# Mozobo/Ocean-Simulation

Measured on AMD Instinct MI355X. Metric: ocean-surface frames/sec (4x1024^2 cascades), higher is better.
Workload: dtype f32; 1 GPU; cfg3: 4 x 1024^2 cascades, displacement + derivatives + Jacobian foam; n=1024, cascades=4, tiles_per_gpu=1, tiles_total=1, schedule=fused (pass A + pass B), parallelism=independent oceans over 1 GPU(s), no collective

## Files before the change

### ocean-simulation_amd/csrc/fftq.hip

```cpp
#include "fft_engine.h"
#include "spectrum_math.h"

namespace ocean {
namespace {

__device__ __forceinline__ float2 hsum(float2 a, float2 b) { return make_float2((a.x + b.x) * 0.5f, (a.y - b.y) * 0.5f); }
__device__ __forceinline__ float2 hdif(float2 a, float2 b) { return make_float2((a.x - b.x) * 0.5f, (a.y + b.y) * 0.5f); }

struct QTex {
    float2 q[3];
};

__device__ __forceinline__ void q_planes(const Planes4& o, const Planes4& om, QTex& a, QTex& b) {
    const float2 h2 = hsum(o.p[1], om.p[1]), h3 = hsum(o.p[2], om.p[2]);
    const float2 a3 = hdif(o.p[2], om.p[2]), h4 = hsum(o.p[3], om.p[3]);
    a.q[0] = o.p[0];
    b.q[0] = om.p[0];
    a.q[1] = make_float2(h2.x - h3.y, h2.y + h3.x);
    b.q[1] = make_float2(h2.x + h3.y, h3.x - h2.y);
    a.q[2] = make_float2(a3.y - h4.y, h4.x - a3.x);
    b.q[2] = make_float2(a3.y + h4.y, a3.x + h4.x);
}

__device__ __forceinline__ void q_fast(float2 h, float4 w, QTex& a, QTex& b) {
    const float c1x = -w.z * w.y, c1y = w.x * w.y;
    a.q[0] = make_float2(c1x * h.x - c1y * h.y, c1x * h.y + c1y * h.x);
    b.q[0] = make_float2(-(c1x * h.x + c1y * h.y), c1x * h.y - c1y * h.x);
    const float s2a = 1.0f - w.x, s2b = 1.0f + w.x;
    a.q[1] = make_float2(s2a * h.x, s2a * h.y);
    b.q[1] = make_float2(s2b * h.x, -s2b * h.y);
    const float kk = w.x * w.x * w.y;
    const float t1 = w.z - kk, t2 = -w.z - kk;
    a.q[2] = make_float2(-t1 * h.y, t1 * h.x);
    b.q[2] = make_float2(t2 * h.y, t2 * h.x);
}

__device__ __forceinline__ float2 q4_minus(const Planes4& o, const Planes4& om, float kz) {
    const float2 a2 = hdif(o.p[1], om.p[1]), a4 = hdif(o.p[3], om.p[3]);
    return make_float2(a2.y + a4.x + kz * o.p[0].y, -a2.x + a4.y - kz * o.p[0].x);
}
__device__ __forceinline__ float2 q4_full(const Planes4& o, const Planes4& om) {
    const float2 a2 = hdif(o.p[1], om.p[1]), a4 = hdif(o.p[3], om.p[3]);
    return make_float2(a2.y + a4.x, -a2.x + a4.y);
}

template <int N>
__device__ __forceinline__ float4 mirror_factors(int x, int y, const WaveBand& wb, float g, float time) {
    const float kx = (float)(x - N / 2) * wb.dk, kz = (float)(y - N / 2) * wb.dk;
    const float kmag = sqrtf(kx * kx + kz * kz);
    if (!(kmag >= wb.lo && kmag <= wb.hi)) return make_float4(1.0f, 0.0f, 1.0f, 0.0f);
    const Phase e = evolve_phase(sqrtf(g * kmag), time);
    return make_float4(e.ex, e.ey, __builtin_amdgcn_rcpf(kmag), 0.0f);
}

__device__ __forceinline__ float2* q_side(const DevView& v, int u) { return v.qside + (size_t)u * 2 * v.n; }

template <int N, bool BAND = false, int WT = 0, bool OFF32 = true>
__global__ __launch_bounds__(N / 4) __attribute__((amdgpu_waves_per_eu(N == 1024 ? 3 : 1, N == 1024 ? 3 : 10))) void
k_pass_aq(DevView v, float time, int items) {
    constexpr int R0 = 4, NJ = N / R0;
    constexpr int IPU = N / 2 + 1;
    using TW = StageTw<N, R0>;
    using E = Engine<N, 4, false, true, R0, TW, kElems>;
    constexpr int T = E::THREADS;
    static_assert(T == NJ && E::R0 == R0, "lane j <-> stage-0 butterfly j");
    constexpr int W = WT ? WT : inter_w(N);
    constexpr int TILES = N / W;
    constexpr int NSL = N / E::RL;
    static_assert(NSL % W == 0, "tile-major emit");
    __shared__ float2 lds[E::LDS_ELEMS];
    __shared__ float2 twl[TW::kLdsEntries];
    TW::load(twl, v.tw, threadIdx.x, T);
    const float2* tws = TW::table(twl, v.tw);
    __shared__ WaveBand band[kMaxCascades];
    if ((int)threadIdx.x < v.C) band[threadIdx.x] = wave_band(v.casc + threadIdx.x * 5);
    const int j = (int)threadIdx.x;
    const int jm = (NJ - j) & (NJ - 1);
    const bool j0 = (j == 0);
    auto rows_of = [&](int it, int& u, int& y1, int& y2) {
        u = it / IPU;
        y1 = it - u * IPU;
        y2 = (N - y1) & (N - 1);
    };
    auto load_pair = [&](int it, float2 (&a)[R0], float2 (&b)[R0]) {
        int u, y1, y2;
        rows_of(it, u, y1, y2);
        const float2* r1 = v.h0k + ((size_t)u * N + y1) * N;
        const float2* r2 = v.h0k + ((size_t)u * N + y2) * N;
#pragma unroll
        for (int r = 0; r < R0; ++r) {
            a[r] = r1[j + r * NJ];
            b[r] = r2[(N - j - r * NJ) & (N - 1)];
        }
    };
    auto unmirror = [&](const float2* mir, float2* out) {
#pragma unroll
        for (int r2 = 0; r2 < R0; ++r2) out[r2] = j0 ? mir[(R0 - r2) & (R0 - 1)] : mir[R0 - 1 - r2];
    };
    auto put = [&](int b, int jb, const float2* x) {
        float2* dst = lds + E::lidx(b, jb * R0);
#pragma unroll
        for (int q = 0; q < R0; ++q) dst[E::loff(q, 1)] = x[q];
    };
    float2 A[R0], B[R0], An[R0], Bn[R0];
    int it = blockIdx.x;
    if (it < items) load_pair(it, A, B);
    __syncthreads();
    for (; it < items; it += gridDim.x) {
        const int next = it + gridDim.x;
        if (next < items) load_pair(next, An, Bn);
        int u, y1, y2;
        rows_of(it, u, y1, y2);
        const WaveBand wb = band[(u + v.c0) % v.C];
        const bool self = (y1 == y2);
        const Win wunit = make_win(v.tplane + (size_t)u * TILES * N * W, 0);
        float2 g[6][R0];
        {
            float2 mir[3][R0];
#pragma unroll
            for (int r = 0; r < R0; ++r) {
                const float4 f = mirror_factors<N>(j + r * NJ, y1, wb, v.gravity, time);
                const float4 wd = make_float4((float)(j + r * NJ - N / 2) * wb.dk, f.z, (float)(y1 - N / 2) * wb.dk, 0.0f);
                const float2 h = evolve_h(make_float4(A[r].x, A[r].y, B[r].x, -B[r].y), Phase{f.x, f.y});
                QTex qa, qb;
                if (y1 != 0 && !(r == 0 && j0)) {
                    q_fast(h, wd, qa, qb);
                } else {
                    const float4 wm = make_float4((j0 && r == 0) ? wd.x : -wd.x, wd.y, y1 ? -wd.z : wd.z, wd.w);
                    const Planes4 o = planes_of(h, wd), om = planes_of(make_float2(h.x, -h.y), wm);
                    q_planes(o, om, qa, qb);
                    if (y1 == 0) qb.q[2] = q4_full(o, om);
                    if (r == 0 && j0) {
                        float2* side = q_side(v, u);
                        side[y1] = q4_minus(o, om, wd.z);
                        side[y2] = q4_minus(om, o, wm.z);
// ... 297 lines not shown
            const int mm = jj + q * NSL;
            if (b == 6) {
                if (y1 == 0) q_side(v, u)[N + mm] = val;
                return;
            }
            if (b >= 3 && self) return;
            const int p = b >= 3 ? b - 3 : b;
            const int y = b >= 3 ? y2 : y1;
            if constexpr (OFF32) {
                const unsigned e = (unsigned)p * (unsigned)v.inter_stride + ((unsigned)u * TILES * N + (unsigned)y) * W +
                                   (unsigned)(jj / W) * N * W + (unsigned)(jj % W) + (unsigned)q * (NSL / W) * N * W;
                *(float2*)((char*)v.tplane + (store_off_t)(e * 8u)) = val;
            } else {
                float2* dst = v.tplane + (size_t)p * v.inter_stride + ((size_t)u * TILES * N + y) * W +
                              (size_t)(jj / W) * N * W + (jj % W);
                dst[(size_t)q * (NSL / W) * N * W] = val;
            }
        };
        E::template stages_from<1>(lds, tws, emit, live);
        __syncthreads();
    }
}

template <int N, bool BAND = false, int WT = 0, bool DC = false>
__global__ __launch_bounds__((WT ? WT : b3_w(N)) * N / kElems) void k_pass_bq(DevView v, int items) {
    using CT = ColTile<N, WT ? WT : b3_w(N)>;
    using E = typename CT::E;
    using TW = typename CT::TW;
    constexpr int W = CT::W;
    constexpr int T = CT::T;
    constexpr int RL = CT::RL;
    constexpr int TILE = W * N;
    constexpr bool kKeepLds = (E::LDS_ELEMS + TW::kLdsEntries + kElems * T + N) * 8 <= 160 * 1024;
    __shared__ float2 lds[E::LDS_ELEMS];
    __shared__ float2 twl[TW::kLdsEntries];
    __shared__ float2 keep_lds[kKeepLds ? kElems * T : 1];
    __shared__ float dks[kMaxCascades];
    __shared__ float2 d0s[N];
    constexpr int DPL = (N + T - 1) / T;
    TW::load(twl, v.tw, threadIdx.x, T);
    const float2* tws = TW::table(twl, v.tw);
    if ((int)threadIdx.x < v.C) dks[threadIdx.x] = wave_band(v.casc + threadIdx.x * 5).dk;
    const int lb = CT::lane_b(), lj = CT::lane_j();
    const int toff = lj * W + lb;
    const int voff16 = (lj * N + lb) * 16;

    float2 keep_reg[kKeepLds ? 1 : kElems];
    auto kput = [&](int i, float2 x) {
        if constexpr (kKeepLds) keep_lds[i * T + threadIdx.x] = x;
        else keep_reg[i] = x;
    };
    auto kget = [&](int i) -> float2 {
        if constexpr (kKeepLds) return keep_lds[i * T + threadIdx.x];
        else return keep_reg[i];
    };
    const int bt0 = v.x0 / W, bnt = v.nx / W;
    constexpr int G = DC ? 1 : 32;
    const bool grp = G > 1 && items % (8 * G) == 0;
    auto full = [&](int item) {
        if (grp) item = (item & ~(8 * G - 1)) + G * (item & 7) + ((item >> 3) & (G - 1));
        return BAND ? (item / bnt) * CT::tiles + bt0 + item % bnt : item;
    };
    auto win16 = [&](const float4* base, int ft) {
        const int u = ft / CT::tiles, x0 = (ft % CT::tiles) * W;
        return make_win(base + (size_t)u * N * N + x0, (unsigned)((N * N - x0) * 16));
    };
    auto load = [&](int item, int p, float2 (&d)[kElems]) {
        const Win w = make_win(v.tplane + (size_t)p * v.inter_stride + (size_t)full(item) * TILE, TILE * 8);
#pragma unroll
        for (int i = 0; i < kElems; ++i)
            d[i] = DC ? bload2<2>(w, toff * 8, CT::in_dy(i) * W * 8) : bload2(w, toff * 8, CT::in_dy(i) * W * 8);
    };

    float2 cur[kElems], nxt[kElems], nx2[kElems], dd[DPL], srow = make_float2(0.0f, 0.0f);
    float kreg[kElems];
    int item = blockIdx.x;
    if (item < items) {
        load(item, 1, cur);
        load(item, 0, nxt);
    }
    __syncthreads();
    for (; item < items; item += gridDim.x) {
        const int ft = full(item);
        const int u = ft / CT::tiles;
        const int x0 = (ft % CT::tiles) * W;
        const float dk = dks[(u + v.c0) % v.C];
        float* foam = v.foam + (size_t)ft * TILE + toff;
        float fb[kElems];
        const bool more = item + (int)gridDim.x < items;
#pragma unroll
        for (int st = 0; st < 4; ++st) {
            if (st == 0) {
                const float2* side = q_side(v, u);
#pragma unroll
                for (int k = 0; k < DPL; ++k)
                    if (k * T + (int)threadIdx.x < N) dd[k] = side[k * T + threadIdx.x];
                if (lj == 0) srow = side[N + x0 + lb];
                load(item, 2, nx2);
            } else if (st == 1) {
#pragma unroll
                for (int r = 0; r < kElems; ++r) {
                    const int y = lj + CT::in_dy(r);
                    const float kz = (float)(y - N / 2) * dk;
                    const float2 c = cur[r], d = d0s[y];
                    nx2[r] = make_float2(d.x - kz * c.y, d.y + kz * c.x);
                }
                if (lj == 0) nx2[0] = srow;
            } else {
                if (st == 2) {
                    const Win rf = make_win(v.foam + (size_t)ft * TILE, TILE * 4);
#pragma unroll
                    for (int m = 0; m < kElems / RL; ++m)
#pragma unroll
                        for (int q = 0; q < RL; ++q) fb[m * RL + q] = bload1(rf, toff * 4, CT::out_dy(m, q) * W * 4);
                }
                if (more) load(item + gridDim.x, st == 2 ? 1 : 0, nx2);
            }
            const Win wd = win16(v.disp, ft), wt = win16(v.turb, ft), wv = win16(v.deriv, ft);
            auto emit = [&](int m, int q, float2 val) {
                const int i = m * RL + q;
// ... 27 lines not shown
            }
#pragma unroll
            for (int i = 0; i < kElems; ++i) {
                if (st == 1) {
                    cur[i] = nx2[i];
                } else {
                    cur[i] = nxt[i];
                    nxt[i] = nx2[i];
                }
            }
            __syncthreads();
        }
    }
}

template <class K>
int grid_q(K kernel, int threads, int items) {
    const int g = device_cus() * resident_per_cu((const void*)kernel, threads);
    return items < g ? items : g;
}

bool inter_off32(const DevView& v) { return ((size_t)2 * v.inter_stride + v.inter_stride) * 8 <= ((size_t)1 << 32); }

template <int N, bool BAND = false, int WT = 0, bool OFF32 = true>
hipError_t go_aq(const DevView& v, float t, hipStream_t s) {
    if constexpr (WT == 0) {
        if (v.tile_w != inter_w(N)) return go_aq<N, BAND, 4, OFF32>(v, t, s);
    }
    if constexpr (!BAND) {
        if (v.nx != N) return go_aq<N, true, WT, OFF32>(v, t, s);
    }
    if constexpr (OFF32) {
        if (!inter_off32(v)) return go_aq<N, BAND, WT, false>(v, t, s);
    }
    constexpr int T = N / 4;
    const int items = v.units * (N / 2 + 1);
    const int g = grid_q(k_pass_aq<N, BAND, WT, OFF32>, T, items);
    launch((k_pass_aq<N, BAND, WT, OFF32>), dim3(g), dim3(T), 0, s, v, t, items);
    return hipGetLastError();
}

template <int N, bool BAND = false>
hipError_t go_a3q(const DevView& v, float t, hipStream_t s) {
    if constexpr (!BAND) {
        if (v.nx != N) return go_a3q<N, true>(v, t, s);
    }
    constexpr int T = N / 4;
    const int total = v.units * N;
    const int g = grid_q(k_pass_a3q<N, BAND>, T, total);
    launch((k_pass_a3q<N, BAND>), dim3(g), dim3(T), 0, s, v, t, total);
    return hipGetLastError();
}

template <int N, bool BAND = false, int WT = 0, bool DC = false>
hipError_t go_bq(const DevView& v, hipStream_t s) {
    if constexpr (WT == 0) {
        if (v.tile_w != inter_w(N)) return go_bq<N, BAND, 4, DC>(v, s);
    }
    if constexpr (!BAND) {
        if (v.nx != N) return go_bq<N, true, WT, DC>(v, s);
    }
    if constexpr (!DC) {
        if (v.disp_cached) return go_bq<N, BAND, WT, true>(v, s);
    }
    constexpr int W = WT ? WT : b3_w(N);
    constexpr int T = W * N / kElems;
    const int items = v.units * (v.nx / W);
    const int g = grid_q(k_pass_bq<N, BAND, WT, DC>, T, items);
    launch((k_pass_bq<N, BAND, WT, DC>), dim3(g), dim3(T), 0, s, v, items);
    return hipGetLastError();
}

}

bool pass_q_supported(int n, int planes) { return planes == 4 && (n == 512 || n == 1024 || n == 4096); }

hipError_t launch_pass_a_q(const DevView& v, float t, hipStream_t s) {
    if (!pass_q_supported(v.n, v.planes) || !v.qside) return hipErrorInvalidValue;
    if (v.xstr == 2) {
        if (v.n != 4096 || v.x0 != 0 || v.nx != v.n / 2 || !v.h0k) return hipErrorInvalidValue;
        constexpr int T = 4096 / 4;
        const int items = v.units * (4096 / 2 + 1);
        if (inter_off32(v)) {
            const int g = grid_q(k_pass_a3pp<4096, true>, T, items);
            launch((k_pass_a3pp<4096, true>), dim3(g), dim3(T), 0, s, v, t, items);
        } else {
            const int g = grid_q(k_pass_a3pp<4096, false>, T, items);
            launch((k_pass_a3pp<4096, false>), dim3(g), dim3(T), 0, s, v, t, items);
        }
        return hipGetLastError();
    }
    switch (v.n) {
        case 512: return v.h0k ? go_aq<512>(v, t, s) : hipErrorInvalidValue;
        case 1024: return v.h0k ? go_aq<1024>(v, t, s) : hipErrorInvalidValue;
        case 4096: return go_a3q<4096>(v, t, s);
    }
    return hipErrorInvalidValue;
}

hipError_t launch_pass_b_q(const DevView& v, hipStream_t s) {
    if (!pass_q_supported(v.n, v.planes) || v.n > 1024 || !v.qside) return hipErrorInvalidValue;
    return v.n == 512 ? go_bq<512>(v, s) : go_bq<1024>(v, s);
}

}
```

### ocean-simulation_amd/csrc/ocean_abi.cpp

```cpp
#include <cxxabi.h>
#include <hip/hip_runtime.h>

#include <cmath>
#include <cstdio>
#include <cstdlib>
#include <cstring>
#include <new>
#include <algorithm>
#include <map>
#include <memory>
#include <mutex>
#include <tuple>
#include <string>
#include <vector>

#include "fft_core.h"
#include "device_scope.h"
#include "ocean_internal.h"

namespace {

thread_local std::string g_last_error;

int fail(int code, const std::string& msg) {
    g_last_error = msg;
    return code;
}

int hip_fail(hipError_t e, const char* what) {
    return fail(OCEAN_E_DEVICE, std::string(what) + ": " + hipGetErrorString(e));
}

#define OCEAN_HIP(call)                                   \
    do {                                                  \
        hipError_t _e = (call);                           \
        if (_e != hipSuccess) return hip_fail(_e, #call); \
    } while (0)

struct TimedLaunch {
    int kind;
    hipEvent_t a, b;
// ... 102 lines not shown
            sl->tstart = a;
            sl->tdone = b;
        }
        free_slots.pop_back();
        *out = sl;
        return hipSuccess;
    }
    void give(StageSlot* sl) {
        std::lock_guard<std::mutex> lk(mu);
        free_slots.push_back(sl);
    }
};

struct ocean_options {
    int q = 1;
    int a4 = 1;
    long chunk_mib = 192;
    int c4_bands = 0;
    long op_chunk_mib = 0;
    int tile_w = 0;
    int disp_cached = -1;
    int grid_tile = 0;
    int vel_nt = 0;

    static ocean_options from_env() {
        ocean_options o;
        if (const char* e = std::getenv("OCEAN_Q")) o.q = std::atoi(e);
        if (const char* e = std::getenv("OCEAN_A4")) o.a4 = std::atoi(e);
        if (const char* e = std::getenv("OCEAN_CHUNK_MIB")) o.chunk_mib = std::max(0L, std::atol(e));
        if (const char* e = std::getenv("OCEAN_C4_BANDS")) o.c4_bands = std::max(0, std::atoi(e));
        if (const char* e = std::getenv("OCEAN_OP_CHUNK_MIB")) o.op_chunk_mib = std::max(0L, std::atol(e));
        if (const char* e = std::getenv("OCEAN_TILE_W")) o.tile_w = std::max(0, std::atoi(e));
        if (const char* e = std::getenv("OCEAN_DISP_CACHED")) o.disp_cached = std::strcmp(e, "auto") ? std::atoi(e) != 0 : -1;
        if (const char* e = std::getenv("OCEAN_GRID_TILE")) o.grid_tile = std::atoi(e);
        if (const char* e = std::getenv("OCEAN_VEL_NT")) o.vel_nt = std::atoi(e) != 0;
        return o;
    }
};

struct ocean_ctx {
    int device = 0;
    int n = 0, logn = 0, C = 0, T = 0, P = 4;
    uint32_t flags = 0;
    hipStream_t stream = nullptr;
    float2* noise = nullptr;
    float4* h0 = nullptr;
    float2* h0k = nullptr;
    bool h0k_valid = false;
    bool h0_conj = false;
    ocean_options opt;
    size_t inter_units = 0;
    int band_x0 = 0, band_nx = 0;
    int col_par = -1;
    int tile_w = 8;
    float4* waves = nullptr;
    float2* plane[4] = {nullptr, nullptr, nullptr, nullptr};
    float4* disp = nullptr;
    float4* deriv = nullptr;
    float4* turb = nullptr;
    float4* normal = nullptr;
    float4* vel = nullptr;
    float2* vplane = nullptr;
    float2* tw = nullptr;
    float* casc = nullptr;
    float2* tplane = nullptr;
    float* foam = nullptr;
    float2* qside = nullptr;
    float4* deriv_mips = nullptr;
    float4* turb_mips = nullptr;
    size_t mip_chain = 0;
    hipStream_t copy_stream = nullptr;
    std::shared_ptr<StagePool> stage_pool;
    bool readback_timing = false;
    ocean::SpectrumParams params{};
    ocean::SpectrumParams staged_params{};
    float staged_casc[5 * ocean::kMaxCascades] = {};
    bool params_set = false;
    std::vector<bool> noise_set;
    bool spectrum_ready = false;
    bool timing = false;
    std::vector<hipEvent_t> event_pool;
    std::vector<TimedLaunch> pending;
    double kind_ms[3] = {0, 0, 0};
    long long kind_count[3] = {0, 0, 0};
    const void* kind_kernel[3] = {nullptr, nullptr, nullptr};
    static constexpr size_t kMaxPending = 2048;

    size_t texels() const { return (size_t)n * n; }
    size_t units() const { return (size_t)T * C; }

// ... 140 lines not shown
    return nullptr;
}

int slice_ptr(ocean_ctx* ctx, int tex, int tile, int cascade, size_t bytes, char** out) {
    size_t eb = 0, slices = 0;
    void* base = tex_ptr(ctx, tex, &eb, &slices);
    if (tex < OCEAN_TEX_NOISE || tex > OCEAN_TEX_VELOCITY) return fail(OCEAN_E_INVALID_ARG, "unknown texture id");
    if (!base) return fail(OCEAN_E_INVALID_ARG, "texture not allocated for this context's flags");
    if (tile < 0 || tile >= ctx->T) return fail(OCEAN_E_INVALID_ARG, "tile out of range");
    if (tex != OCEAN_TEX_NOISE && (cascade < 0 || cascade >= ctx->C))
        return fail(OCEAN_E_INVALID_ARG, "cascade out of range");
    const size_t slice_bytes = ctx->texels() * eb;
    if (bytes != slice_bytes)
        return fail(OCEAN_E_INVALID_ARG, "byte count " + std::to_string(bytes) + " != slice size " +
                                             std::to_string(slice_bytes));
    const size_t slice = tex == OCEAN_TEX_NOISE ? (size_t)tile : (size_t)tile * ctx->C + cascade;
    *out = static_cast<char*>(base) + slice * slice_bytes;
    return OCEAN_OK;
}

void free_all(ocean_ctx* c) {
    void* ptrs[] = {c->noise, c->h0, c->h0k, c->waves, c->plane[0], c->disp, c->deriv,
                    c->turb,  c->normal, c->tw,    c->casc,     c->tplane, c->foam, c->deriv_mips, c->turb_mips,
                    c->qside, c->vel, c->vplane};
    for (void* p : ptrs)
        if (p) (void)hipFree(p);
    for (auto& t : c->pending) {
        (void)hipEventDestroy(t.a);
        (void)hipEventDestroy(t.b);
    }
    for (auto e : c->event_pool) (void)hipEventDestroy(e);
    if (c->copy_stream) (void)hipStreamDestroy(c->copy_stream);
    if (c->stream) (void)hipStreamDestroy(c->stream);
}

}

namespace {
int chunk_units(const ocean_ctx* ctx, int planes);
int q_planes(const ocean_ctx* ctx) { return ctx->n >= 2048 ? 4 : 3; }
}

extern "C" {

const char* ocean_last_error(void) { return g_last_error.c_str(); }

int ocean_abi_version(void) { return OCEAN_ABI_VERSION; }
// ... 47 lines not shown
    auto alloc = [&](void** p, size_t bytes) -> bool {
        if (hipMalloc(p, bytes) != hipSuccess) return false;
        return hipMemset(*p, 0, bytes) == hipSuccess;
    };
    const size_t tex = c->texels(), U = c->units();
    bool ok = hipStreamCreateWithFlags(&c->stream, hipStreamNonBlocking) == hipSuccess;
    ok = ok && alloc((void**)&c->noise, tex * c->T * 8);
    ok = ok && alloc((void**)&c->h0, tex * U * 16);
    if (ocean::pass_a4_supported(n, c->P)) ok = ok && alloc((void**)&c->h0k, tex * U * 8);
    ok = ok && alloc((void**)&c->waves, tex * U * 16);
    ok = ok && alloc((void**)&c->plane[0], tex * U * 8 * c->P);
    if (ok)
        for (int p = 1; p < c->P; ++p) c->plane[p] = c->plane[0] + (size_t)p * tex * U;
    ok = ok && alloc((void**)&c->disp, tex * U * 16);
    if (c->P == 4) {
        ok = ok && alloc((void**)&c->deriv, tex * U * 16);
        ok = ok && alloc((void**)&c->turb, tex * U * 16);
        ok = ok && alloc((void**)&c->foam, tex * U * 4);
    }
    c->inter_units = (size_t)std::max(chunk_units(c, c->P),
                                      ocean::pass_q_supported(n, c->P) ? chunk_units(c, q_planes(c)) : 1);
    ok = ok && alloc((void**)&c->tplane, tex * c->inter_units * 8 * c->P);
    if (ocean::pass_q_supported(n, c->P)) ok = ok && alloc((void**)&c->qside, c->inter_units * 2 * n * 8);
    if (flags & OCEAN_F_NORMALS) ok = ok && alloc((void**)&c->normal, tex * U * 16);
    if (flags & OCEAN_F_MIPS) {
        for (int l = 1; (n >> l) >= 1; ++l) c->mip_chain += (size_t)(n >> l) * (n >> l);
        ok = ok && alloc((void**)&c->deriv_mips, c->mip_chain * U * 16);
        ok = ok && alloc((void**)&c->turb_mips, c->mip_chain * U * 16);
    }
    if (flags & OCEAN_F_VELOCITY) {
        ok = ok && alloc((void**)&c->vel, tex * U * 16);
        ok = ok && alloc((void**)&c->vplane, tex * U * 8 * 2);
    }
    const size_t tw_entries = (size_t)n + 128 + ocean::stage_twiddle_entries(n);
    ok = ok && alloc((void**)&c->tw, tw_entries * 8);
    ok = ok && alloc((void**)&c->casc, 5 * 4 * 5);
    if (!ok) {
        std::string msg = std::string("device allocation failed: ") + hipGetErrorString(hipGetLastError());
        free_all(c);
        delete c;
        return fail(OCEAN_E_OUT_OF_MEMORY, msg);
    }
    std::vector<float2> tw(tw_entries);
    for (int m = 0; m < n; ++m) {
        const double a = 2.0 * M_PI * (double)m / (double)n;
        tw[m] = make_float2((float)std::cos(a), (float)std::sin(a));
// ... 67 lines not shown
    ctx->noise_set[tile] = true;
    return OCEAN_OK;
}

int ocean_generate_noise_device(ocean_ctx* ctx, uint64_t seed) {
    OCEAN_ENTER(ctx);
    const ocean::DevView v = ctx->view();
    OCEAN_HIP(ocean::launch_noise(v, seed, ctx->stream));
    OCEAN_HIP(hipStreamSynchronize(ctx->stream));
    for (int t = 0; t < ctx->T; ++t) ctx->noise_set[t] = true;
    return OCEAN_OK;
}

int ocean_generate_noise(ocean_ctx* ctx, uint64_t seed) {
    OCEAN_ENTER(ctx);
    std::vector<float> host(ctx->texels() * 2);
    for (int t = 0; t < ctx->T; ++t) {
        ocean::generate_noise_host(ctx->n, seed + (uint64_t)t, host.data());
        if (int r = ocean_set_noise(ctx, t, host.data())) return r;
    }
    return OCEAN_OK;
}

int ocean_init_spectrum(ocean_ctx* ctx) {
    OCEAN_ENTER(ctx);
    if (!ctx->params_set) return fail(OCEAN_E_STATE, "ocean_set_params must precede ocean_init_spectrum");
    for (int t = 0; t < ctx->T; ++t)
        if (!ctx->noise_set[t]) return fail(OCEAN_E_STATE, "noise not set for tile " + std::to_string(t));
    OCEAN_HIP(hipMemcpyAsync(ctx->casc, ctx->staged_casc, (size_t)ctx->C * 5 * 4, hipMemcpyHostToDevice, ctx->stream));
    OCEAN_HIP(hipStreamSynchronize(ctx->stream));
    ctx->params = ctx->staged_params;
    const ocean::DevView v = ctx->view();
    if (int r = timed(ctx, 2, [&] { return ocean::launch_init_spectrum(v, ctx->params, ctx->stream); },
                      "init_spectrum"))
        return r;
    if (int r = timed(ctx, 2, [&] { return ocean::launch_conjugate(v, ctx->stream); }, "conjugate")) return r;
    ctx->spectrum_ready = true;
    ctx->h0k_valid = ctx->h0k != nullptr;
    ctx->h0_conj = true;
    return OCEAN_OK;
}

int ocean_reset_foam(ocean_ctx* ctx) {
    OCEAN_ENTER(ctx);
    if (ctx->turb) OCEAN_HIP(hipMemsetAsync(ctx->turb, 0, ctx->texels() * ctx->units() * 16, ctx->stream));
    if (ctx->foam) OCEAN_HIP(hipMemsetAsync(ctx->foam, 0, ctx->texels() * ctx->units() * 4, ctx->stream));
    if (ctx->turb_mips) OCEAN_HIP(hipMemsetAsync(ctx->turb_mips, 0, ctx->mip_chain * ctx->units() * 16, ctx->stream));
    return OCEAN_OK;
}

int ocean_evolve(ocean_ctx* ctx, float time) {
    OCEAN_ENTER(ctx);
    if (!ctx->spectrum_ready) return fail(OCEAN_E_STATE, "ocean_init_spectrum must precede ocean_evolve");
    const ocean::DevView v = ctx->view();
    return timed(ctx, 2, [&] { return ocean::launch_evolve(v, time, ctx->stream); }, "evolve");
}

namespace {
int ifft_unit_planes(ocean_ctx* ctx, const ocean::DevView& v, float2* base0, int ups, int kind_rows, int kind_cols) {
    const size_t up_elems = ctx->texels();
    if (ctx->n == 4096) {
        const long mib = ctx->opt.op_chunk_mib > 0 ? ctx->opt.op_chunk_mib : 256;
        const int k = (int)std::max<size_t>(1, ((size_t)mib << 20) / (up_elems * 8));
// ... 150 lines not shown
    const int U = (int)ctx->units(), K = std::min(chunk_units(ctx, q ? q_planes(ctx) : ctx->P), (int)ctx->inter_units);
    v.disp_cached = disp_fits_cache(ctx, q, K);
    for (int u0 = 0; u0 < U; u0 += K) {
        const ocean::DevView c = (K >= U) ? v : sub_view(v, u0, std::min(K, U - u0), ctx->inter_units < ctx->units());
        if (q && ctx->n >= 2048) {
            if (int r = timed(ctx, 0, [&] { return ocean::launch_pass_a_q(c, time, ctx->stream); }, "pass_a")) return r;
            const int nb = c4_bands(ctx, c.nx);
            if (nb == 1) {
                if (int r = timed(ctx, 1, [&] { return ocean::launch_pass_c4q(c, ctx->stream); }, "pass_c")) return r;
                continue;
            }
            const int w = c.nx / nb;
            for (int u = 0; u < c.units; ++u)
                for (int b = 0; b < nb; ++b) {
                    ocean::DevView cb = sub_view(c, u, 1);
                    cb.x0 = c.x0 + b * w;
                    cb.nx = (b == nb - 1) ? c.nx - b * w : w;
                    if (int r = timed(ctx, 1, [&] { return ocean::launch_pass_c4q(cb, ctx->stream); }, "pass_c"))
                        return r;
                }
            continue;
        }
        if (q) {
            if (int r = timed(ctx, 0, [&] { return ocean::launch_pass_a_q(c, time, ctx->stream); }, "pass_a")) return r;
            if (int r = timed(ctx, 1, [&] { return ocean::launch_pass_b_q(c, ctx->stream); }, "pass_b")) return r;
            continue;
        }
        if (int r = timed(ctx, 0, [&] {
                if (ctx->opt.a4 && ctx->h0k_valid && ocean::pass_a4_supported(ctx->n, ctx->P))
                    return ocean::launch_pass_a_v4(c, time, ctx->stream);
                return ocean::launch_pass_a_v3(c, time, ctx->stream);
            }, "pass_a"))
            return r;
        const int nb = c4_bands(ctx, c.nx);
        if (nb > 1) {
            const int w = c.nx / nb;
            for (int u = 0; u < c.units; ++u)
                for (int b = 0; b < nb; ++b) {
                    ocean::DevView cb = sub_view(c, u, 1);
                    cb.x0 = c.x0 + b * w;
                    cb.nx = (b == nb - 1) ? c.nx - b * w : w;
                    if (int r = timed(ctx, 1, [&] { return ocean::launch_pass_c4(cb, ctx->stream); }, "pass_c"))
                        return r;
                }
            continue;
        }
        if (int r = timed(ctx, 1, [&] {
                if (ocean::pass_c4_supported(ctx->n)) return ocean::launch_pass_c4(c, ctx->stream);
// ... 777 lines not shown
```

### ocean-simulation_amd/csrc/ocean_internal.h

```cpp
#pragma once

#include <hip/hip_ext.h>
#include <hip/hip_runtime.h>
#include <stdint.h>

#include "ocean/ocean.h"

namespace ocean {

struct LaunchEvents {
    hipEvent_t start, stop;
    bool launched;
};
LaunchEvents*& launch_events();
const void*& last_kernel();

template <class F, class... Args>
inline void launch(F kernel, dim3 grid, dim3 block, uint32_t shmem, hipStream_t s, Args... args) {
    last_kernel() = (const void*)kernel;
    LaunchEvents* e = launch_events();
    hipExtLaunchKernelGGL(kernel, grid, block, shmem, s, e && !e->launched ? e->start : nullptr,
                          e ? e->stop : nullptr, 0, args...);
    if (e) e->launched = true;
}
// ... 30 lines not shown
    float4* deriv_mips;
    float4* turb_mips;
    size_t mip_chain;
    int x0, nx;
    int c0;
    int xstr, xpar;
    bool disp_cached;
};

struct SpectrumParams {
    float wind_speed, wind_dir_x, wind_dir_y, gravity, fetch, depth;
};

int resident_per_cu(const void* kernel, int threads);
int device_cus();

hipError_t launch_init_spectrum(const DevView& v, const SpectrumParams& p, hipStream_t s);
hipError_t launch_conjugate(const DevView& v, hipStream_t s);
hipError_t launch_evolve(const DevView& v, float t, hipStream_t s);
hipError_t launch_fill(const DevView& v, hipStream_t s);
hipError_t launch_foam_import(const DevView& v, hipStream_t s);
hipError_t launch_noise(const DevView& v, uint64_t seed, hipStream_t s);
hipError_t launch_h0k_extract(const DevView& v, hipStream_t s);

size_t stage_twiddle_entries(int n);
hipError_t launch_ifft_rows_v2(const DevView& v, float2* base, int ups, hipStream_t s);
hipError_t launch_ifft_cols_v2(const DevView& v, float2* base, int ups, hipStream_t s);
hipError_t launch_ifft_fold(const DevView& v, float2* planes, int ups, int part, hipStream_t s);

hipError_t launch_pass_a_v3(const DevView& v, float t, hipStream_t s);
hipError_t launch_pass_b_v3(const DevView& v, hipStream_t s);
hipError_t launch_mips(const DevView& v, hipStream_t s);
hipError_t launch_extract_height(const float4* disp_slice, float* dst, size_t texels, hipStream_t s);
hipError_t launch_sample_world(const DevView& v, int tile, const float* pts, int count, float* out, hipStream_t s);
hipError_t launch_query_surface(const DevView& v, int tile, int mode, int iterations, const float* pts, int count,
                                float* out, hipStream_t s);
bool grid_tile_supported(int tile_w);
hipError_t launch_surface_grid(const DevView& v, int tile, int mode, int iterations, float lod, float x0, float z0,
                               float dx, float dz, int nx, int ny, int tile_w, float* out, hipStream_t s);
int body_segment_width(int probes);
hipError_t launch_body_buoyancy(const DevView& v, int tile, int mode, int iterations, const float* hull, int probes,
                                const float* bodies, int count, float* out, hipStream_t s);
hipError_t launch_evolve_velocity(const DevView& v, float2* scratch, float t, hipStream_t s);
hipError_t launch_pack_velocity(const DevView& v, const float2* scratch, float4* vel, bool streamed, hipStream_t s);
hipError_t launch_query_velocity(const DevView& v, const float4* vel, int tile, int iterations, const float* pts,
                                 int count, float* out, hipStream_t s);

bool pass_c4_supported(int n);
hipError_t launch_pass_c4(const DevView& v, hipStream_t s);
bool pass_a4_supported(int n, int planes);
hipError_t launch_pass_a_v4(const DevView& v, float t, hipStream_t s);
bool pass_q_supported(int n, int planes);
hipError_t launch_pass_a_q(const DevView& v, float t, hipStream_t s);
hipError_t launch_pass_b_q(const DevView& v, hipStream_t s);
hipError_t launch_pass_c4q(const DevView& v, hipStream_t s);

}
```

### ocean-simulation_amd/csrc/spectrum.hip

```cpp
#include "ocean_internal.h"
#include "spectrum_math.h"

namespace ocean {
namespace {

struct Sp {
    float U, g, F, D, wdx, wdy;
};


__device__ __forceinline__ float sp_pow(float a, float b) { return (float)pow((double)a, (double)b); }
__device__ __forceinline__ float sp_exp(float a) { return (float)exp((double)a); }
__device__ __forceinline__ float sp_log(float a) { return (float)log((double)a); }
__device__ __forceinline__ float sp_tanh(float a) { return (float)tanh((double)a); }
__device__ __forceinline__ float sp_cosh(float a) { return (float)cosh((double)a); }
__device__ __forceinline__ float sp_cos(float a) { return (float)cos((double)a); }
__device__ __forceinline__ float sp_atan2(float a, float b) { return (float)atan2((double)a, (double)b); }

__device__ __forceinline__ float tma_correction(const Sp& p, float w) {
    float wh = w * sqrtf(p.D / p.g);
    if (wh <= 1.0f) return 0.5f * wh * wh;
    if (wh < 2.0f) return 1.0f - 0.5f * (2.0f - wh) * (2.0f - wh);
    return 1.0f;
}
// ... 143 lines not shown
            ++k;
            return (float)(mix64(key + k * 0x9E3779B97F4A7C15ull) >> 40) * (1.0f / 16777216.0f);
        };
        float g[2];
        for (int c = 0; c < 2; ++c) {
            float v1, v2, q;
            do {
                v1 = 2.0f * uniform() - 1.0f;
                v2 = 2.0f * uniform() - 1.0f;
                q = v1 * v1 + v2 * v2;
            } while (q >= 1.0f || q == 0.0f);
            g[c] = v1 * sqrtf(-2.0f * logf(q) / q);
        }
        noise[i] = make_float2(g[0], g[1]);
    }
}

__global__ __launch_bounds__(256) void k_h0k_extract(DevView v) {
    const size_t total = (size_t)v.n * v.n * v.units;
    for (size_t i = blockIdx.x * (size_t)blockDim.x + threadIdx.x; i < total; i += (size_t)gridDim.x * blockDim.x)
        v.h0k[i] = *reinterpret_cast<const float2*>(&v.h0[i]);
}

unsigned grid_for(size_t total) {
    size_t g = (total + 255) / 256;
    return (unsigned)(g < 16384 ? (g == 0 ? 1 : g) : 16384);
}

}

hipError_t launch_noise(const DevView& v, uint64_t seed, hipStream_t s) {
    const size_t total = (size_t)v.n * v.n * v.T;
    launch(k_noise, dim3(grid_for(total)), dim3(256), 0, s, const_cast<float2*>(v.noise), v.n, v.T, seed);
    return hipGetLastError();
}

hipError_t launch_init_spectrum(const DevView& v, const SpectrumParams& sp, hipStream_t s) {
    Sp p{sp.wind_speed, sp.gravity, sp.fetch, sp.depth, sp.wind_dir_x, sp.wind_dir_y};
    launch(k_init_spectrum, dim3(grid_for((size_t)v.n * v.n * v.units)), dim3(256), 0, s, v, p);
    return hipGetLastError();
}

hipError_t launch_conjugate(const DevView& v, hipStream_t s) {
    launch(k_conjugate, dim3(grid_for((size_t)v.n * v.n * v.units)), dim3(256), 0, s, v);
    return hipGetLastError();
}

hipError_t launch_evolve(const DevView& v, float t, hipStream_t s) {
    launch(k_evolve, dim3(grid_for((size_t)v.n * v.n * v.units)), dim3(256), 0, s, v, t);
    return hipGetLastError();
}

hipError_t launch_foam_import(const DevView& v, hipStream_t s) {
    launch(k_foam_import, dim3(grid_for((size_t)v.n * v.n * v.units)), dim3(256), 0, s, v);
    return hipGetLastError();
}

hipError_t launch_h0k_extract(const DevView& v, hipStream_t s) {
    if (!v.h0k) return hipErrorInvalidValue;
    launch(k_h0k_extract, dim3(grid_for((size_t)v.n * v.n * v.units)), dim3(256), 0, s, v);
    return hipGetLastError();
}

hipError_t launch_fill(const DevView& v, hipStream_t s) {
    launch(k_fill, dim3(grid_for((size_t)v.n * v.n * v.units)), dim3(256), 0, s, v);
    return hipGetLastError();
}

}
```

Baseline: 12100 frames/s.

## Prune all-zero spectrum rows from fused q-pass FFT schedule

At spectrum init, a new kernel scans h0k to find for each cascade the largest row distance from the center that holds any nonzero coefficient. Pass A then iterates over a compacted table of live row pairs instead of all N/2+1. Pass B masks loads of dead rows to a zero out-of-range offset and zeroes the matching side data. This skips FFT work on rows the band-limited cascades never populate. It adds a host sync at init and only switches on when at least one eighth of the rows are dead.

```diff
diff --git a/ocean-simulation_amd/csrc/fftq.hip b/ocean-simulation_amd/csrc/fftq.hip
--- a/ocean-simulation_amd/csrc/fftq.hip
+++ b/ocean-simulation_amd/csrc/fftq.hip
@@ -9,6 +9,21 @@
 
 struct QTex {
     float2 q[3];
+};
+
+typedef __attribute__((address_space(4))) const int cint_t;
+template <bool PRUNE>
+struct AqTable {};
+template <>
+struct AqTable<true> {
+    const int* tab;
+    int ubase;
+};
+template <bool PRUNE>
+struct BqExtents {};
+template <>
+struct BqExtents<true> {
+    const int* ext;
 };
 
 __device__ __forceinline__ void q_planes(const Planes4& o, const Planes4& om, QTex& a, QTex& b) {
@@ -55,9 +70,9 @@
 
 __device__ __forceinline__ float2* q_side(const DevView& v, int u) { return v.qside + (size_t)u * 2 * v.n; }
 
-template <int N, bool BAND = false, int WT = 0, bool OFF32 = true>
+template <int N, bool BAND = false, int WT = 0, bool OFF32 = true, bool PRUNE = false>
 __global__ __launch_bounds__(N / 4) __attribute__((amdgpu_waves_per_eu(N == 1024 ? 3 : 1, N == 1024 ? 3 : 10))) void
-k_pass_aq(DevView v, float time, int items) {
+k_pass_aq(DevView v, float time, int items, AqTable<PRUNE> pt) {
     constexpr int R0 = 4, NJ = N / R0;
     constexpr int IPU = N / 2 + 1;
     using TW = StageTw<N, R0>;
@@ -77,14 +92,24 @@
     const int j = (int)threadIdx.x;
     const int jm = (NJ - j) & (NJ - 1);
     const bool j0 = (j == 0);
-    auto rows_of = [&](int it, int& u, int& y1, int& y2) {
-        u = it / IPU;
-        y1 = it - u * IPU;
+    static_assert(!(PRUNE && BAND), "column-band contexts run the dense schedule");
+    auto key_of = [&](int it) {
+        if constexpr (PRUNE) return (int)((const cint_t*)pt.tab)[it];
+        else return it;
+    };
+    auto rows_of = [&](int key, int& u, int& y1, int& y2) {
+        if constexpr (PRUNE) {
+            u = (key >> 16) - pt.ubase;
+            y1 = key & 0xffff;
+        } else {
+            u = key / IPU;
+            y1 = key - u * IPU;
+        }
         y2 = (N - y1) & (N - 1);
     };
-    auto load_pair = [&](int it, float2 (&a)[R0], float2 (&b)[R0]) {
+    auto load_pair = [&](int key, float2 (&a)[R0], float2 (&b)[R0]) {
         int u, y1, y2;
-        rows_of(it, u, y1, y2);
+        rows_of(key, u, y1, y2);
         const float2* r1 = v.h0k + ((size_t)u * N + y1) * N;
         const float2* r2 = v.h0k + ((size_t)u * N + y2) * N;
 #pragma unroll
@@ -104,13 +129,22 @@
     };
     float2 A[R0], B[R0], An[R0], Bn[R0];
     int it = blockIdx.x;
-    if (it < items) load_pair(it, A, B);
+    int key = 0;
+    if (it < items) {
+        key = key_of(it);
+        load_pair(key, A, B);
+    }
     __syncthreads();
     for (; it < items; it += gridDim.x) {
         const int next = it + gridDim.x;
-        if (next < items) load_pair(next, An, Bn);
+        int nkey = 0;
+        if (next < items) {
+            nkey = key_of(next);
+            load_pair(nkey, An, Bn);
+        }
         int u, y1, y2;
-        rows_of(it, u, y1, y2);
+        rows_of(PRUNE ? key : it, u, y1, y2);
+        if (PRUNE) key = nkey;
         const WaveBand wb = band[(u + v.c0) % v.C];
         const bool self = (y1 == y2);
         const Win wunit = make_win(v.tplane + (size_t)u * TILES * N * W, 0);
@@ -454,8 +488,9 @@
     }
 }
 
-template <int N, bool BAND = false, int WT = 0, bool DC = false>
-__global__ __launch_bounds__((WT ? WT : b3_w(N)) * N / kElems) void k_pass_bq(DevView v, int items) {
+template <int N, bool BAND = false, int WT = 0, bool DC = false, bool PRUNE = false>
+__global__ __launch_bounds__((WT ? WT : b3_w(N)) * N / kElems) void k_pass_bq(DevView v, int items, BqExtents<PRUNE> pe) {
+    static_assert(!(PRUNE && BAND), "column-band contexts run the dense schedule");
     using CT = ColTile<N, WT ? WT : b3_w(N)>;
     using E = typename CT::E;
     using TW = typename CT::TW;
@@ -497,8 +532,23 @@
         const int u = ft / CT::tiles, x0 = (ft % CT::tiles) * W;
         return make_win(base + (size_t)u * N * N + x0, (unsigned)((N * N - x0) * 16));
     };
+    auto extent_of = [&](int u) {
+        if constexpr (PRUNE) return (int)((const cint_t*)pe.ext)[u];
+        else return N / 2;
+    };
+    constexpr int kDeadOff = 0x40000000;
+    auto is_live = [&](int y, int m) { return m >= 0 && (unsigned)(y - (N / 2 - m)) <= (unsigned)(2 * m); };
     auto load = [&](int item, int p, float2 (&d)[kElems]) {
         const Win w = make_win(v.tplane + (size_t)p * v.inter_stride + (size_t)full(item) * TILE, TILE * 8);
+        if constexpr (PRUNE) {
+            const int m = extent_of(full(item) / CT::tiles);
+#pragma unroll
+            for (int i = 0; i < kElems; ++i) {
+                const int vo = is_live(lj + CT::in_dy(i), m) ? toff * 8 : kDeadOff;
+                d[i] = DC ? bload2<2>(w, vo, CT::in_dy(i) * W * 8) : bload2(w, vo, CT::in_dy(i) * W * 8);
+            }
+            return;
+        }
 #pragma unroll
         for (int i = 0; i < kElems; ++i)
             d[i] = DC ? bload2<2>(w, toff * 8, CT::in_dy(i) * W * 8) : bload2(w, toff * 8, CT::in_dy(i) * W * 8);
@@ -524,10 +574,15 @@
         for (int st = 0; st < 4; ++st) {
             if (st == 0) {
                 const float2* side = q_side(v, u);
-#pragma unroll
-                for (int k = 0; k < DPL; ++k)
-                    if (k * T + (int)threadIdx.x < N) dd[k] = side[k * T + threadIdx.x];
-                if (lj == 0) srow = side[N + x0 + lb];
+                const int m = extent_of(u);
+#pragma unroll
+                for (int k = 0; k < DPL; ++k) {
+                    const int y = k * T + (int)threadIdx.x;
+                    if (PRUNE) dd[k] = make_float2(0.0f, 0.0f);
+                    if (y < N && (!PRUNE || is_live(y, m))) dd[k] = side[y];
+                }
+                if (PRUNE) srow = make_float2(0.0f, 0.0f);
+                if (lj == 0 && m == N / 2) srow = side[N + x0 + lb];
                 load(item, 2, nx2);
             } else if (st == 1) {
 #pragma unroll
@@ -601,21 +656,30 @@
 
 bool inter_off32(const DevView& v) { return ((size_t)2 * v.inter_stride + v.inter_stride) * 8 <= ((size_t)1 << 32); }
 
-template <int N, bool BAND = false, int WT = 0, bool OFF32 = true>
-hipError_t go_aq(const DevView& v, float t, hipStream_t s) {
+template <int N, bool BAND = false, int WT = 0, bool OFF32 = true, bool PRUNE = false>
+hipError_t go_aq(const DevView& v, float t, hipStream_t s, const PruneView* pv) {
     if constexpr (WT == 0) {
-        if (v.tile_w != inter_w(N)) return go_aq<N, BAND, 4, OFF32>(v, t, s);
-    }
-    if constexpr (!BAND) {
-        if (v.nx != N) return go_aq<N, true, WT, OFF32>(v, t, s);
+        if (v.tile_w != inter_w(N)) return go_aq<N, BAND, 4, OFF32, PRUNE>(v, t, s, pv);
+    }
+    if constexpr (!BAND && !PRUNE) {
+        if (v.nx != N) return pv ? hipErrorInvalidValue : go_aq<N, true, WT, OFF32>(v, t, s, nullptr);
     }
     if constexpr (OFF32) {
-        if (!inter_off32(v)) return go_aq<N, BAND, WT, false>(v, t, s);
+        if (!inter_off32(v)) return go_aq<N, BAND, WT, false, PRUNE>(v, t, s, pv);
+    }
+    if constexpr (!BAND && !PRUNE) {
+        if (pv) return go_aq<N, false, WT, OFF32, true>(v, t, s, pv);
     }
     constexpr int T = N / 4;
-    const int items = v.units * (N / 2 + 1);
-    const int g = grid_q(k_pass_aq<N, BAND, WT, OFF32>, T, items);
-    launch((k_pass_aq<N, BAND, WT, OFF32>), dim3(g), dim3(T), 0, s, v, t, items);
+    if constexpr (PRUNE) {
+        if (pv->items <= 0) return hipErrorInvalidValue;
+        const int g = grid_q(k_pass_aq<N, BAND, WT, OFF32, true>, T, pv->items);
+        launch((k_pass_aq<N, BAND, WT, OFF32, true>), dim3(g), dim3(T), 0, s, v, t, pv->items, AqTable<true>{pv->tab, pv->ubase});
+    } else {
+        const int items = v.units * (N / 2 + 1);
+        const int g = grid_q(k_pass_aq<N, BAND, WT, OFF32>, T, items);
+        launch((k_pass_aq<N, BAND, WT, OFF32>), dim3(g), dim3(T), 0, s, v, t, items, AqTable<false>{});
+    }
     return hipGetLastError();
 }
 
@@ -631,22 +695,27 @@
     return hipGetLastError();
 }
 
-template <int N, bool BAND = false, int WT = 0, bool DC = false>
-hipError_t go_bq(const DevView& v, hipStream_t s) {
+template <int N, bool BAND = false, int WT = 0, bool DC = false, bool PRUNE = false>
+hipError_t go_bq(const DevView& v, hipStream_t s, const PruneView* pv) {
     if constexpr (WT == 0) {
-        if (v.tile_w != inter_w(N)) return go_bq<N, BAND, 4, DC>(v, s);
-    }
-    if constexpr (!BAND) {
-        if (v.nx != N) return go_bq<N, true, WT, DC>(v, s);
+        if (v.tile_w != inter_w(N)) return go_bq<N, BAND, 4, DC, PRUNE>(v, s, pv);
+    }
+    if constexpr (!BAND && !PRUNE) {
+        if (v.nx != N) return pv ? hipErrorInvalidValue : go_bq<N, true, WT, DC>(v, s, nullptr);
     }
     if constexpr (!DC) {
-        if (v.disp_cached) return go_bq<N, BAND, WT, true>(v, s);
+        if (v.disp_cached) return go_bq<N, BAND, WT, true, PRUNE>(v, s, pv);
+    }
+    if constexpr (!BAND && !PRUNE) {
+        if (pv) return go_bq<N, false, WT, DC, true>(v, s, pv);
     }
     constexpr int W = WT ? WT : b3_w(N);
     constexpr int T = W * N / kElems;
     const int items = v.units * (v.nx / W);
-    const int g = grid_q(k_pass_bq<N, BAND, WT, DC>, T, items);
-    launch((k_pass_bq<N, BAND, WT, DC>), dim3(g), dim3(T), 0, s, v, items);
+    const int g = grid_q(k_pass_bq<N, BAND, WT, DC, PRUNE>, T, items);
+    BqExtents<PRUNE> pe;
+    if constexpr (PRUNE) pe.ext = pv->ext;
+    launch((k_pass_bq<N, BAND, WT, DC, PRUNE>), dim3(g), dim3(T), 0, s, v, items, pe);
     return hipGetLastError();
 }
 
@@ -654,8 +723,9 @@
 
 bool pass_q_supported(int n, int planes) { return planes == 4 && (n == 512 || n == 1024 || n == 4096); }
 
-hipError_t launch_pass_a_q(const DevView& v, float t, hipStream_t s) {
+hipError_t launch_pass_a_q(const DevView& v, float t, hipStream_t s, const PruneView* pv) {
     if (!pass_q_supported(v.n, v.planes) || !v.qside) return hipErrorInvalidValue;
+    if (pv && (v.n > 1024 || v.xstr != 1 || v.nx != v.n)) return hipErrorInvalidValue;
     if (v.xstr == 2) {
         if (v.n != 4096 || v.x0 != 0 || v.nx != v.n / 2 || !v.h0k) return hipErrorInvalidValue;
         constexpr int T = 4096 / 4;
@@ -670,16 +740,17 @@
         return hipGetLastError();
     }
     switch (v.n) {
-        case 512: return v.h0k ? go_aq<512>(v, t, s) : hipErrorInvalidValue;
-        case 1024: return v.h0k ? go_aq<1024>(v, t, s) : hipErrorInvalidValue;
+        case 512: return v.h0k ? go_aq<512>(v, t, s, pv) : hipErrorInvalidValue;
+        case 1024: return v.h0k ? go_aq<1024>(v, t, s, pv) : hipErrorInvalidValue;
         case 4096: return go_a3q<4096>(v, t, s);
     }
     return hipErrorInvalidValue;
 }
 
-hipError_t launch_pass_b_q(const DevView& v, hipStream_t s) {
+hipError_t launch_pass_b_q(const DevView& v, hipStream_t s, const PruneView* pv) {
     if (!pass_q_supported(v.n, v.planes) || v.n > 1024 || !v.qside) return hipErrorInvalidValue;
-    return v.n == 512 ? go_bq<512>(v, s) : go_bq<1024>(v, s);
-}
-
-}
+    if (pv && v.nx != v.n) return hipErrorInvalidValue;
+    return v.n == 512 ? go_bq<512>(v, s, pv) : go_bq<1024>(v, s, pv);
+}
+
+}
diff --git a/ocean-simulation_amd/csrc/ocean_abi.cpp b/ocean-simulation_amd/csrc/ocean_abi.cpp
--- a/ocean-simulation_amd/csrc/ocean_abi.cpp
+++ b/ocean-simulation_amd/csrc/ocean_abi.cpp
@@ -17,6 +17,7 @@
 #include "fft_core.h"
 #include "device_scope.h"
 #include "ocean_internal.h"
+#include "prune_items.h"
 
 namespace {
 
@@ -165,6 +166,7 @@
     int disp_cached = -1;
     int grid_tile = 0;
     int vel_nt = 0;
+    int prune = 1;
 
     static ocean_options from_env() {
         ocean_options o;
@@ -177,6 +179,7 @@
         if (const char* e = std::getenv("OCEAN_DISP_CACHED")) o.disp_cached = std::strcmp(e, "auto") ? std::atoi(e) != 0 : -1;
         if (const char* e = std::getenv("OCEAN_GRID_TILE")) o.grid_tile = std::atoi(e);
         if (const char* e = std::getenv("OCEAN_VEL_NT")) o.vel_nt = std::atoi(e) != 0;
+        if (const char* e = std::getenv("OCEAN_PRUNE")) o.prune = std::atoi(e);
         return o;
     }
 };
@@ -209,6 +212,9 @@
     float2* tplane = nullptr;
     float* foam = nullptr;
     float2* qside = nullptr;
+    int* prune_dev = nullptr;
+    ocean::PruneItems prune;
+    bool prune_ready = false;
     float4* deriv_mips = nullptr;
     float4* turb_mips = nullptr;
     size_t mip_chain = 0;
@@ -395,7 +401,7 @@
 void free_all(ocean_ctx* c) {
     void* ptrs[] = {c->noise, c->h0, c->h0k, c->waves, c->plane[0], c->disp, c->deriv,
                     c->turb,  c->normal, c->tw,    c->casc,     c->tplane, c->foam, c->deriv_mips, c->turb_mips,
-                    c->qside, c->vel, c->vplane};
+                    c->qside, c->vel, c->vplane, c->prune_dev};
     for (void* p : ptrs)
         if (p) (void)hipFree(p);
     for (auto& t : c->pending) {
@@ -489,6 +495,8 @@
                                       ocean::pass_q_supported(n, c->P) ? chunk_units(c, q_planes(c)) : 1);
     ok = ok && alloc((void**)&c->tplane, tex * c->inter_units * 8 * c->P);
     if (ocean::pass_q_supported(n, c->P)) ok = ok && alloc((void**)&c->qside, c->inter_units * 2 * n * 8);
+    if (c->opt.prune && c->qside && c->h0k && n <= 1024 && U < (size_t)ocean::kPruneMaxUnits)
+        ok = ok && alloc((void**)&c->prune_dev, (U + U * (n / 2 + 1)) * sizeof(int));
     if (flags & OCEAN_F_NORMALS) ok = ok && alloc((void**)&c->normal, tex * U * 16);
     if (flags & OCEAN_F_MIPS) {
         for (int l = 1; (n >> l) >= 1; ++l) c->mip_chain += (size_t)(n >> l) * (n >> l);
@@ -602,6 +610,27 @@
     return OCEAN_OK;
 }
 
+namespace {
+int rebuild_prune(ocean_ctx* ctx) {
+    ctx->prune_ready = false;
+    if (!ctx->prune_dev) return OCEAN_OK;
+    const ocean::DevView v = ctx->view();
+    const int U = (int)ctx->units();
+    OCEAN_HIP(ocean::launch_live_extent(v, ctx->prune_dev, ctx->stream));
+    std::vector<int> ext((size_t)U);
+    OCEAN_HIP(hipMemcpyAsync(ext.data(), ctx->prune_dev, (size_t)U * sizeof(int), hipMemcpyDeviceToHost, ctx->stream));
+    OCEAN_HIP(hipMemsetAsync(ctx->qside, 0, ctx->inter_units * 2 * ctx->n * 8, ctx->stream));
+    OCEAN_HIP(hipStreamSynchronize(ctx->stream));
+    ctx->prune.build(ext.data(), U, ctx->n);
+    if (!ctx->prune.items.empty())
+        OCEAN_HIP(hipMemcpyAsync(ctx->prune_dev + U, ctx->prune.items.data(), ctx->prune.items.size() * sizeof(int),
+                                 hipMemcpyHostToDevice, ctx->stream));
+    OCEAN_HIP(hipStreamSynchronize(ctx->stream));
+    ctx->prune_ready = true;
+    return OCEAN_OK;
+}
+}
+
 int ocean_init_spectrum(ocean_ctx* ctx) {
     OCEAN_ENTER(ctx);
     if (!ctx->params_set) return fail(OCEAN_E_STATE, "ocean_set_params must precede ocean_init_spectrum");
@@ -618,7 +647,7 @@
     ctx->spectrum_ready = true;
     ctx->h0k_valid = ctx->h0k != nullptr;
     ctx->h0_conj = true;
-    return OCEAN_OK;
+    return rebuild_prune(ctx);
 }
 
 int ocean_reset_foam(ocean_ctx* ctx) {
@@ -815,8 +844,22 @@
             continue;
         }
         if (q) {
-            if (int r = timed(ctx, 0, [&] { return ocean::launch_pass_a_q(c, time, ctx->stream); }, "pass_a")) return r;
-            if (int r = timed(ctx, 1, [&] { return ocean::launch_pass_b_q(c, ctx->stream); }, "pass_b")) return r;
+            constexpr long kPruneMinDeadShare = 8;
+            ocean::PruneView pv{};
+            bool prune = ctx->prune_ready && !ctx->prune.dense && c.nx == ctx->n;
+            if (prune) {
+                int first = 0;
+                ctx->prune.chunk(u0, c.units, &first, &pv.items);
+                pv.tab = ctx->prune_dev + U + first;
+                pv.ubase = u0;
+                pv.ext = ctx->prune_dev + u0;
+                prune = (long)pv.items * kPruneMinDeadShare <= (long)c.units * (ctx->n / 2 + 1) * (kPruneMinDeadShare - 1);
+            }
+            const ocean::PruneView* pp = prune ? &pv : nullptr;
+            if (!prune || pv.items > 0)
+                if (int r = timed(ctx, 0, [&] { return ocean::launch_pass_a_q(c, time, ctx->stream, pp); }, "pass_a"))
+                    return r;
+            if (int r = timed(ctx, 1, [&] { return ocean::launch_pass_b_q(c, ctx->stream, pp); }, "pass_b")) return r;
             continue;
         }
         if (int r = timed(ctx, 0, [&] {
diff --git a/ocean-simulation_amd/csrc/ocean_internal.h b/ocean-simulation_amd/csrc/ocean_internal.h
--- a/ocean-simulation_amd/csrc/ocean_internal.h
+++ b/ocean-simulation_amd/csrc/ocean_internal.h
@@ -76,6 +76,7 @@
 hipError_t launch_foam_import(const DevView& v, hipStream_t s);
 hipError_t launch_noise(const DevView& v, uint64_t seed, hipStream_t s);
 hipError_t launch_h0k_extract(const DevView& v, hipStream_t s);
+hipError_t launch_live_extent(const DevView& v, int* ext, hipStream_t s);
 
 size_t stage_twiddle_entries(int n);
 hipError_t launch_ifft_rows_v2(const DevView& v, float2* base, int ups, hipStream_t s);
@@ -105,8 +106,14 @@
 bool pass_a4_supported(int n, int planes);
 hipError_t launch_pass_a_v4(const DevView& v, float t, hipStream_t s);
 bool pass_q_supported(int n, int planes);
-hipError_t launch_pass_a_q(const DevView& v, float t, hipStream_t s);
-hipError_t launch_pass_b_q(const DevView& v, hipStream_t s);
+struct PruneView {
+    const int* tab;
+    int items;
+    int ubase;
+    const int* ext;
+};
+hipError_t launch_pass_a_q(const DevView& v, float t, hipStream_t s, const PruneView* pv = nullptr);
+hipError_t launch_pass_b_q(const DevView& v, hipStream_t s, const PruneView* pv = nullptr);
 hipError_t launch_pass_c4q(const DevView& v, hipStream_t s);
 
 }
diff --git a/ocean-simulation_amd/csrc/prune_items.h b/ocean-simulation_amd/csrc/prune_items.h
--- /dev/null
+++ b/ocean-simulation_amd/csrc/prune_items.h
@@ -0,0 +1,35 @@
+#pragma once
+
+#include <vector>
+
+namespace ocean {
+
+constexpr int kPruneRowBits = 16;
+constexpr int kPruneMaxUnits = 1 << 15;
+constexpr int prune_pack(int u, int y1) { return (u << kPruneRowBits) | y1; }
+constexpr int prune_unit(int item) { return item >> kPruneRowBits; }
+constexpr int prune_row(int item) { return item & ((1 << kPruneRowBits) - 1); }
+
+struct PruneItems {
+    std::vector<int> pre;
+    std::vector<int> items;
+    bool dense = true;
+
+    void build(const int* ext, int units, int n) {
+        pre.assign((size_t)units + 1, 0);
+        items.clear();
+        dense = true;
+        for (int u = 0; u < units; ++u) {
+            const int m = ext[u] < -1 ? -1 : (ext[u] > n / 2 ? n / 2 : ext[u]);
+            dense = dense && m == n / 2;
+            for (int i = n / 2 - m; i <= n / 2; ++i) items.push_back(prune_pack(u, i));
+            pre[(size_t)u + 1] = (int)items.size();
+        }
+    }
+    void chunk(int u0, int nu, int* first, int* count) const {
+        *first = pre[(size_t)u0];
+        *count = pre[(size_t)u0 + nu] - pre[(size_t)u0];
+    }
+};
+
+}
diff --git a/ocean-simulation_amd/csrc/spectrum.hip b/ocean-simulation_amd/csrc/spectrum.hip
--- a/ocean-simulation_amd/csrc/spectrum.hip
+++ b/ocean-simulation_amd/csrc/spectrum.hip
@@ -189,6 +189,18 @@
         v.h0k[i] = *reinterpret_cast<const float2*>(&v.h0[i]);
 }
 
+__global__ __launch_bounds__(256) void k_live_extent(DevView v, int* ext) {
+    const int n = v.n;
+    const int u = (int)blockIdx.x / n, y = (int)blockIdx.x % n;
+    const float2* row = v.h0k + ((size_t)u * n + y) * n;
+    bool any = false;
+    for (int x = (int)threadIdx.x; x < n; x += (int)blockDim.x) {
+        const float2 h = row[x];
+        any = any || !(h.x == 0.0f) || !(h.y == 0.0f);
+    }
+    if (__syncthreads_or(any) && threadIdx.x == 0) atomicMax(ext + u, y < n / 2 ? n / 2 - y : y - n / 2);
+}
+
 unsigned grid_for(size_t total) {
     size_t g = (total + 255) / 256;
     return (unsigned)(g < 16384 ? (g == 0 ? 1 : g) : 16384);
@@ -229,6 +241,13 @@
     return hipGetLastError();
 }
 
+hipError_t launch_live_extent(const DevView& v, int* ext, hipStream_t s) {
+    if (!v.h0k || !ext) return hipErrorInvalidValue;
+    if (const hipError_t e = hipMemsetAsync(ext, 0xff, (size_t)v.units * sizeof(int), s)) return e;
+    launch(k_live_extent, dim3((unsigned)(v.units * v.n)), dim3(256), 0, s, v, ext);
+    return hipGetLastError();
+}
+
 hipError_t launch_fill(const DevView& v, hipStream_t s) {
     launch(k_fill, dim3(grid_for((size_t)v.n * v.n * v.units)), dim3(256), 0, s, v);
     return hipGetLastError();
```

Measured after the change: 12670 frames/s, median of 6. +4.7%, better.
